# UBC-ECE-Sasha/PIM-compression

Measured on AMD Instinct MI355X. Metric: end-to-end GB/s (compress + decompress) on Silesia-mix; bit-exact ratio parity, higher is better.
Workload: dtype u8; 1 GPU; silesia_mix 8 x 1024 MiB containers in all (BASELINE configs[4]), block_size 32768; containers_this_rank=8, container_bytes=1073741824, block_size=32768, parallelism=whole containers dealt over 1 GPU(s), no collective

## Files before the change

pim-compression_amd/csrc/snappy_k1_stream.hpp:

```cpp
#pragma once

namespace snappy_hip {

#ifdef SNAPPY_EMU
inline unsigned long long g_stream_stats[16] = {0};
#define STREAM_STAT(i) do { if (lane == 0) ++g_stream_stats[i]; } while (0)
#else
#define STREAM_STAT(i) ((void)0)
#endif

#ifdef SNAPPY_PROF
__device__ unsigned long long g_prof[32];
struct StreamProf {
    unsigned long long acc = 0, cnt = 0, last = 0;
};
#define PROF_START() (prof.last = __builtin_readcyclecounter())
#define PROF_LAP(i) do { const unsigned long long now_ = __builtin_readcyclecounter(); if (lane == (i)) { prof.acc += now_ - prof.last; prof.cnt++; } prof.last = now_; } while (0)
#define PROF_WAIT() __builtin_amdgcn_s_waitcnt(0)
#define PROF_FLUSH() do { if (lane < 16) { atomicAdd(&g_prof[lane], prof.acc); atomicAdd(&g_prof[16 + lane], prof.cnt); } } while (0)
#elif defined(SNAPPY_MARK)
struct StreamProf {};
#define PROF_START() asm volatile("; PHASE start")
#define PROF_LAP(i) asm volatile("; PHASE " #i)
#define PROF_WAIT() ((void)0)
#define PROF_FLUSH() ((void)0)
#else
struct StreamProf {};
#define PROF_START() ((void)0)
#define PROF_LAP(i) ((void)0)
#define PROF_WAIT() ((void)0)
#define PROF_FLUSH() ((void)0)
#endif

template <class T, class = void> struct table_gathers_once : std::false_type {};
template <class T> struct table_gathers_once<T, std::void_t<decltype(T::kGathersOnce)>> : std::true_type {};

constexpr uint32_t kStreamRoom = 192;
#ifndef SNAPPY_STREAM_SLOTS_LDS
#define SNAPPY_STREAM_SLOTS_LDS 512
#endif
constexpr uint32_t kStreamSlotsLds = SNAPPY_STREAM_SLOTS_LDS, kStreamSlotsGlobal = 256;
__host__ __device__ constexpr uint32_t stream_scratch_bytes(uint32_t slots) { return 8u * slots; }

struct StreamWindow {
    uint32_t base;
    uint4 a, b;
    uint32_t h0, e0;
};

__device__ __forceinline__ void stream_load_window(StreamWindow& w, const uint8_t* __restrict__ blk, uint32_t base, uint32_t last16,
                                                   uint32_t lane)
{
    w.base = base;
    const uint32_t q = base + lane;
    w.a = ld128(blk + (q < last16 ? q : last16));
    w.b = ld128(blk + (q + 16u < last16 ? q + 16u : last16));
}
__device__ __forceinline__ void stream_hash_window(StreamWindow& w, uint32_t shift)
{
    const uint32_t prod = w.a.x * kHashMul;
    w.h0 = prod >> shift;
    w.e0 = (prod << (32 - shift)) & 0xffff0000u;
}

struct StreamGather {
    uint32_t ent;
    uint4 ka, kb;
    unsigned long long worthm;
};
template <class Table>
__device__ __forceinline__ void stream_issue_gather(StreamGather& g, const Table& table, const StreamWindow& w,
                                                    const uint8_t* __restrict__ blk, uint32_t lane)
{
    const uint32_t mine_l = w.e0 | (w.base + lane);
    g.ent = table.load_lane(w.h0, mine_l);
    const bool worth = !Table::certain_miss(g.ent, mine_l);
    g.worthm = __ballot(worth);
    g.ka = g.kb = make_uint4(0, 0, 0, 0);
    if (worth) {
        const uint8_t* __restrict__ c = blk + (g.ent & 0xffffu);
        g.ka = ld128(c);
        g.kb = ld128(c + 16);
    }
}

#ifdef SNAPPY_EMU
__device__ __forceinline__ uint32_t lds_max_rtn(lds_words_t p, uint32_t v)
{
    const uint32_t old = *p;
    if (v > old) *p = v;
    return old;
}
#else
__device__ __forceinline__ uint32_t lds_max_rtn(lds_words_t p, uint32_t v)
{
    return __hip_atomic_fetch_max((__attribute__((address_space(3))) uint32_t*)p, v, __ATOMIC_RELAXED, __HIP_MEMORY_SCOPE_WAVEFRONT);
}
#endif

struct StreamDup {
    uint32_t j1 = 0;
    uint32_t extj = 0;
    unsigned long long nf = 0;
    unsigned long long hitj = 0;
    unsigned long long deep = 0;
    unsigned long long cx = 0;
};

template <uint32_t kSlots>
__device__ __forceinline__ void stream_analyse(StreamDup& d, const StreamWindow& w, lds_bytes_t scratch, uint32_t lane)
{
    lds_words_t tab = (lds_words_t)scratch;
    const uint32_t sa = w.h0 & (kSlots - 1u);
    const uint32_t sb = kSlots + ((w.h0 >> 5) & (kSlots - 1u));
#ifdef SNAPPY_EMU
    static const bool unordered = getenv("EMU_LDS_UNORDERED") != nullptr;
    uint32_t oa = 0, ob = 0;
    if (unordered) {
        oa = lds_max_rtn(tab + sa, lane + 1u);
        ob = lds_max_rtn(tab + sb, lane + 1u);
    } else {
        for (uint32_t turn = 0; turn < kWave; ++turn) {
            if (lane == turn) {
                oa = lds_max_rtn(tab + sa, lane + 1u);
                ob = lds_max_rtn(tab + sb, lane + 1u);
            }
            __builtin_amdgcn_wave_barrier();
        }
    }
#else
    const uint32_t oa = lds_max_rtn(tab + sa, lane + 1u);
    const uint32_t ob = lds_max_rtn(tab + sb, lane + 1u);
#endif
    __builtin_amdgcn_wave_barrier();
    tab[sa] = 0;
    tab[sb] = 0;
    __builtin_amdgcn_wave_barrier();
    const uint32_t ja = oa - 1u, jb = ob - 1u;
    d = StreamDup();
    if (__ballot((oa && ja >= lane) || (ob && jb >= lane))) {
        STREAM_STAT(7);
        d.cx = dup_slot_lanes(scratch, w.h0, lane);
        for (uint32_t i = lane; i < 2u * kSlots; i += kWave) tab[i] = 0;
        __builtin_amdgcn_wave_barrier();
        return;
    }
    const uint32_t ha = (uint32_t)__shfl((int)w.h0, (int)(ja & 63u));
    const uint32_t hb = (uint32_t)__shfl((int)w.h0, (int)(jb & 63u));
    const unsigned long long OA = __ballot(oa != 0), OB = __ballot(ob != 0);
    const unsigned long long MA = OA & __ballot(ha == w.h0), MB = OB & __ballot(hb == w.h0);
    const bool ma = __builtin_amdgcn_inverse_ballot_w64(MA);
    d.j1 = ma ? ja : jb;
    d.nf = MA | MB;
    d.cx = OA & OB & ~d.nf;
    if (d.nf) {
        const uint32_t jl = d.j1 & 63u;
        const uint32_t xj = (uint32_t)__shfl((int)w.a.x, (int)jl);
        const uint32_t e1 = (uint32_t)__shfl((int)w.a.y, (int)jl) ^ w.a.y;
        const uint32_t e2 = (uint32_t)__shfl((int)w.a.z, (int)jl) ^ w.a.z;
        d.hitj = d.nf & __ballot(xj == w.a.x);
        d.extj = min_u32(min_u32(first_bit(e1), first_bit(e2) | 32u), 64u) >> 3;
        const unsigned long long chained = d.nf | d.cx;
        d.deep = d.nf & __ballot(((uint32_t)(chained >> jl) & 1u) != 0);
    }
}

__device__ __forceinline__ void stream_walk(uint32_t advv, uint32_t clv, uint32_t& t, unsigned long long& V, unsigned long long& COV)
{
#ifdef SNAPPY_EMU
    for (;;) {
        const uint32_t l = t & 63u;
        V |= 1ull << l;
        const uint32_t a = (uint32_t)__builtin_amdgcn_readlane((int)advv, (int)l);
        const uint32_t c = (uint32_t)__builtin_amdgcn_readlane((int)clv, (int)l);
        if (c) COV |= ((1ull << c) - 1ull) << l;
        const uint32_t nt = t + a;
        const bool carry = nt < t;
        t = nt;
        if (carry) break;
    }
#else
    uint32_t a, c;
    unsigned long long m;
    asm volatile(
        "1:\n"
        "  s_bitset1_b64 %[V], %[t]\n"
        "  v_readlane_b32 %[a], %[advv], %[t]\n"
        "  v_readlane_b32 %[c], %[clv], %[t]\n"
        "  s_bfm_b64 %[m], %[c], %[t]\n"
        "  s_or_b64 %[COV], %[COV], %[m]\n"
        "  s_add_u32 %[t], %[t], %[a]\n"
        "  s_cbranch_scc1 2f\n"
        "  s_bitset1_b64 %[V], %[t]\n"
        "  v_readlane_b32 %[a], %[advv], %[t]\n"
        "  v_readlane_b32 %[c], %[clv], %[t]\n"
        "  s_bfm_b64 %[m], %[c], %[t]\n"
        "  s_or_b64 %[COV], %[COV], %[m]\n"
        "  s_add_u32 %[t], %[t], %[a]\n"
        "  s_cbranch_scc1 2f\n"
        "  s_bitset1_b64 %[V], %[t]\n"
        "  v_readlane_b32 %[a], %[advv], %[t]\n"
        "  v_readlane_b32 %[c], %[clv], %[t]\n"
        "  s_bfm_b64 %[m], %[c], %[t]\n"
        "  s_or_b64 %[COV], %[COV], %[m]\n"
        "  s_add_u32 %[t], %[t], %[a]\n"
        "  s_cbranch_scc1 2f\n"
        "  s_bitset1_b64 %[V], %[t]\n"
        "  v_readlane_b32 %[a], %[advv], %[t]\n"
        "  v_readlane_b32 %[c], %[clv], %[t]\n"
        "  s_bfm_b64 %[m], %[c], %[t]\n"
        "  s_or_b64 %[COV], %[COV], %[m]\n"
        "  s_add_u32 %[t], %[t], %[a]\n"
        "  s_cbranch_scc0 1b\n"
        "2:\n"
        : [t] "+s"(t), [V] "+s"(V), [COV] "+s"(COV), [a] "=&s"(a), [c] "=&s"(c), [m] "=&s"(m)
        : [advv] "v"(advv), [clv] "v"(clv)
        : "scc");
#endif
}

#ifndef SNAPPY_EMU
__device__ __forceinline__ unsigned long long uni64(unsigned long long v)
{
    return (unsigned long long)uni((uint32_t)v) | ((unsigned long long)uni((uint32_t)(v >> 32)) << 32);
}
#else
__device__ __forceinline__ unsigned long long uni64(unsigned long long v) { return v; }
#endif

__device__ __forceinline__ uint32_t stream_past(uint32_t dist, unsigned long long inter, uint32_t land)
{
    if (land >= kWave || ((inter >> land) & 1ull)) return 0;
    return (uint32_t)__builtin_amdgcn_readlane((int)dist, (int)land);
}

__device__ __forceinline__ bool has_run_of_34(unsigned long long m)
{
    unsigned long long r = m & (m >> 1);
    r &= r >> 2;
    r &= r >> 4;
    r &= r >> 8;
    r &= r >> 16;
    return (r & (m >> 32) & (m >> 33)) != 0;
}

template <class Table>
__device__ __forceinline__ void stream_put(const Table& table, uint32_t x, uint32_t pos, uint32_t shift, uint32_t lane)
{
    const uint32_t prod = x * kHashMul;
    if constexpr (Table::kCollectiveStore)
        table.store_masked(1ull, prod >> shift, pos, lane);
    else
        table.put(prod >> shift, ((prod << (32 - shift)) & 0xffff0000u) | pos, lane);
}
template <class Table>
__device__ __forceinline__ void stream_store(const Table& table, const StreamWindow& w, unsigned long long m, uint32_t lane)
{
    if constexpr (Table::kCollectiveStore) {
        table.store_masked(m, w.h0, w.base + lane, lane);
    } else {
        if (__builtin_amdgcn_inverse_ballot_w64(m)) table.store_lane(w.h0, w.e0 | (w.base + lane));
        __builtin_amdgcn_wave_barrier();
    }
}

__device__ __forceinline__ void stream_emit(uint8_t* __restrict__ dst, const uint8_t* __restrict__ blk, uint32_t& op, uint32_t& next_emit,
                                            uint32_t base, uint32_t x0, uint32_t ent, uint32_t extv, unsigned long long H,
                                            unsigned long long COV, bool by_copy, uint32_t r_out, bool long_copy, uint32_t ip,
                                            uint32_t long_cand, uint32_t long_len, uint32_t lane)
{
    if (H) emit_segment(dst, blk, op, next_emit, base, x0, ent, extv, H, COV, by_copy, r_out, lane);
    if (long_copy) {
        if (ip > next_emit) op = emit_literal_windowed(dst, op, blk, next_emit, ip - next_emit, base, x0, lane);
        op = emit_copy(dst, op, ip - long_cand, long_len, lane);
        next_emit = ip + long_len;
    }
}

struct SoloMate {
    static constexpr bool kAnalysesInPlace = true;
    __device__ __forceinline__ void begin(uint32_t, uint32_t, uint32_t) {}
    __device__ __forceinline__ void drain(uint32_t&, uint32_t&, uint32_t) {}
    template <uint32_t kSlots>
    __device__ __forceinline__ void analysis(StreamDup& d, const StreamWindow& w, lds_bytes_t scratch, uint32_t lane)
    {
        stream_analyse<kSlots>(d, w, scratch, lane);
    }
    __device__ __forceinline__ void emit(uint8_t* __restrict__ dst, const uint8_t* __restrict__ blk, uint32_t& op, uint32_t& next_emit,
                                         uint32_t base, uint32_t x0, uint32_t ent, uint32_t extv, unsigned long long H,
                                         unsigned long long COV, bool by_copy, uint32_t r_out, bool long_copy, uint32_t ip,
                                         uint32_t long_cand, uint32_t long_len, uint32_t lane)
    {
        stream_emit(dst, blk, op, next_emit, base, x0, ent, extv, H, COV, by_copy, r_out, long_copy, ip, long_cand, long_len, lane);
    }
};

template <class Table, uint32_t kSlots, class Mate>
__device__ __forceinline__ void stream_run(const uint8_t* __restrict__ blk, uint32_t avail, uint32_t n, uint32_t shift,
                                           uint8_t* __restrict__ dst, const Table table, uint32_t lane, lds_bytes_t dup_scratch,
                                           ParseState& ps, StreamProf& prof, Mate& mate)
{
    const uint32_t limit = n - kInputMargin;
    const uint32_t last16 = avail - 16u;
    uint32_t ip = ps.ip, skip = ps.skip, op = ps.op, next_emit = ps.next_emit;
    mate.begin(op, next_emit, lane);

    for (;;) {
        StreamWindow cur, nxt;
        stream_load_window(cur, blk, ip & ~63u, last16, lane);
        stream_hash_window(cur, shift);
        StreamGather g;
        stream_issue_gather(g, table, cur, blk, lane);
        __builtin_amdgcn_sched_barrier(0);
        stream_load_window(nxt, blk, cur.base + 64u, last16, lane);
        StreamDup dup;
        mate.template analysis<kSlots>(dup, cur, dup_scratch, lane);
        PROF_LAP(0);
        bool restart = false;

        for (;;) {
            const uint32_t r0 = ip - cur.base;
            const uint32_t b_in = 64u - skip;
            PROF_WAIT();
            PROF_LAP(1);

            unsigned long long hitm = __ballot(g.ka.x == cur.a.x) & g.worthm;
            const uint32_t t1 = min_u32(first_bit(g.ka.y ^ cur.a.y), first_bit(g.ka.z ^ cur.a.z) | 32u);
            const uint32_t t2 = min_u32(first_bit(g.ka.w ^ cur.a.w), first_bit(g.kb.x ^ cur.b.x) | 32u) | 64u;
            const uint32_t t3 = min_u32(first_bit(g.kb.y ^ cur.b.y), first_bit(g.kb.z ^ cur.b.z) | 32u) | 128u;
            uint32_t extv = min_u32(min_u32(t1, t2), min_u32(t3, 192u)) >> 3;
            uint32_t ent = g.ent & 0xffffu;
            const unsigned long long pend = dup.nf & __ballot(dup.j1 >= r0);
            const unsigned long long satm = hitm & __ballot(extv == 24u);
            unsigned long long stopm = pend | dup.cx | satm;
            const unsigned long long above_r0 = ~0ull << r0;
            const unsigned long long inter = hitm | stopm;
            const unsigned long long up = (lane < 63u) ? (inter >> (lane + 1u)) : 0ull;
            const uint32_t dist = up ? (uint32_t)__builtin_ctzll(up) + 1u : 64u - lane;
            const bool stopl = __builtin_amdgcn_inverse_ballot_w64(stopm);
            const bool hitl = __builtin_amdgcn_inverse_ballot_w64(hitm);
            const uint32_t clt = hitl ? 4u + extv : 0u;
            const bool hitjl = __builtin_amdgcn_inverse_ballot_w64(dup.hitj);
            const uint32_t clj = hitjl ? 4u + dup.extj : 0u;
            const uint32_t land_t = lane + clt, land_j = lane + clj;
            const uint32_t dist_t = (uint32_t)__shfl((int)dist, (int)(land_t & 63u));
            const uint32_t dist_j = (uint32_t)__shfl((int)dist, (int)(land_j & 63u));
            const bool plain_t = land_t < 64u && !((inter >> (land_t & 63u)) & 1ull);
            const bool plain_j = land_j < 64u && !((inter >> (land_j & 63u)) & 1ull);
            const uint32_t advt = hitl ? clt + (plain_t ? dist_t : 0u) : dist;
            const uint32_t advj = hitjl ? clj + (plain_j ? dist_j : 0u) : dist;
            const unsigned long long satjm = dup.hitj & __ballot(dup.extj == 8u);
            uint32_t clv = stopl ? 0u : clt;
            uint32_t advv = stopl ? 64u : advt;
            PROF_LAP(2);

            unsigned long long V = 0, COV = 0;
            uint32_t t = r0 - 64u;
            uint32_t r_out = 0;
            bool long_copy = false;
            uint32_t long_cand = 0, long_len = 0;
            for (;;) {
                t = uni(t);
                stream_walk(advv, clv, t, V, COV);
                const uint32_t s = 63u - (uint32_t)__builtin_clzll(V);
                if (!((stopm >> s) & 1ull)) {
                    r_out = t + 64u;
                    break;
                }
                PROF_LAP(3);
                STREAM_STAT(3);
                const unsigned long long bit_s = 1ull << s;
                const unsigned long long below_s = bit_s - 1ull;
                const unsigned long long interior_s = COV & ~(V & hitm & below_s);
                uint32_t how = 0;
                uint32_t j = 0;
                if (pend & bit_s) {
                    j = (uint32_t)__builtin_amdgcn_readlane((int)dup.j1, (int)s);
                    const unsigned long long not_inserted = interior_s & (interior_s >> 1);
                    if (!((not_inserted >> j) & 1ull)) how = 1;
                    else if (dup.deep & bit_s) how = 2;
                }
                if (dup.cx & bit_s) how = 2;
                uint32_t adv_s, cl_s, cand_s = 0, sat_s = 24;
                bool hit_s, more_s;
                if (how == 2) {
                    STREAM_STAT(6);
                    const unsigned long long ins = ((above_r0 & below_s & ~interior_s) | (COV & ~(interior_s >> 1))) & below_s;
                    const uint32_t hs = (uint32_t)__builtin_amdgcn_readlane((int)cur.h0, (int)s);
                    const unsigned long long J = __ballot(cur.h0 == hs) & ins;
                    how = 0;
                    if (J) {
                        j = 63u - (uint32_t)__builtin_clzll(J);
                        hit_s = (uint32_t)__builtin_amdgcn_readlane((int)cur.a.x, (int)s) == (uint32_t)__builtin_amdgcn_readlane((int)cur.a.x, (int)j);
                        const uint32_t e1 = (uint32_t)__builtin_amdgcn_readlane((int)cur.a.y, (int)s) ^ (uint32_t)__builtin_amdgcn_readlane((int)cur.a.y, (int)j);
                        const uint32_t e2 = (uint32_t)__builtin_amdgcn_readlane((int)cur.a.z, (int)s) ^ (uint32_t)__builtin_amdgcn_readlane((int)cur.a.z, (int)j);
                        const uint32_t ext_s = e1 ? ((uint32_t)__builtin_ctz(e1) >> 3) : (e2 ? 4u + ((uint32_t)__builtin_ctz(e2) >> 3) : 8u);
                        cand_s = cur.base + j;
                        sat_s = 8;
                        more_s = hit_s && ext_s == 8u;
                        cl_s = hit_s ? 4u + ext_s : 0u;
                        adv_s = hit_s ? cl_s : (uint32_t)__builtin_amdgcn_readlane((int)dist, (int)s);
                        if (hit_s && !more_s) adv_s += stream_past(dist, hitm | stopm, s + cl_s);
                        how = 3;
                    }
                }
                if (how == 1) {
                    STREAM_STAT(9);
                    hit_s = (dup.hitj & bit_s) != 0;
                    more_s = (satjm & bit_s) != 0;
                    adv_s = (uint32_t)__builtin_amdgcn_readlane((int)advj, (int)s);
                    cl_s = (uint32_t)__builtin_amdgcn_readlane((int)clj, (int)s);
                    cand_s = cur.base + j;
                    sat_s = 8;
                } else if (how == 0) {
                    STREAM_STAT(10);
                    hit_s = (hitm & bit_s) != 0;
                    more_s = (satm & bit_s) != 0;
                    adv_s = (uint32_t)__builtin_amdgcn_readlane((int)advt, (int)s);
                    cl_s = (uint32_t)__builtin_amdgcn_readlane((int)clt, (int)s);
                }
                if (more_s) {
                    STREAM_STAT(8);
                    if (how == 0) cand_s = (uint32_t)__builtin_amdgcn_readlane((int)ent, (int)s);
                    cl_s = 4u + sat_s + match_extend(blk, cand_s + 4u + sat_s, cur.base + s + 4u + sat_s, n, lane);
                    adv_s = cl_s <= 63u ? cl_s + stream_past(dist, hitm | stopm, s + cl_s) : cl_s;
                    if (cl_s > 63u) {
// ... 156 lines not shown
```

pim-compression_amd/csrc/snappy_kernels.hpp:

```cpp
#pragma once
#include <hip/hip_runtime.h>
#include <type_traits>
#include <stdint.h>
#ifdef SNAPPY_EMU
#include <stdio.h>
#include <stdlib.h>
#endif

#include "snappy_device_common.hpp"

namespace snappy_hip {

constexpr uint32_t kMaxTableEntries = 16384;
constexpr uint32_t kHashMul = 0x1e35a7bdu;
constexpr uint32_t kInputMargin = 15;

#if defined(__HIP_DEVICE_COMPILE__)
#define SNAPPY_PIN(x) asm volatile("" : "+v"(x))
#else
#define SNAPPY_PIN(x) ((void)0)
#endif

constexpr uint32_t kBlockOk = 0;
constexpr uint32_t kBlockInvalid = 1;
constexpr uint32_t kRangeOutOfBounds = 2;

__device__ __forceinline__ uint32_t table_entries_for(uint32_t n)
{
    uint32_t ts = 256;
    while (ts < kMaxTableEntries && ts < n) ts <<= 1;
    return ts;
}


__device__ __forceinline__ uint32_t emit_literal(uint8_t* __restrict__ dst, uint32_t op,
                                                 const uint8_t* __restrict__ src, uint32_t len, uint32_t lane)
{
    const uint32_t n = len - 1;
    uint32_t hdr;
    if (n < 60) {
        hdr = 1;
        if (lane == 0) dst[op] = (uint8_t)(n << 2);
    } else {
        const uint32_t cnt = (n < 256u) ? 1u : ((n < 65536u) ? 2u : 3u);
        hdr = 1 + cnt;
        if (lane < hdr)
            dst[op + lane] = (lane == 0) ? (uint8_t)((59 + cnt) << 2) : (uint8_t)(n >> (8 * (lane - 1)));
    }
    uint8_t* d = dst + op + hdr;
    if (len <= kWave) {
        if (lane < len) d[lane] = src[lane];
    } else {
        uint32_t i = 4 * lane;
        for (; i + 4 <= len; i += 4 * kWave) st32(d + i, ld32(src + i));
        for (; i < len; ++i) d[i] = src[i];
    }
    return op + hdr + len;
}

__device__ __forceinline__ uint32_t emit_copy_piece(uint8_t* __restrict__ dst, uint32_t op, uint32_t off,
                                                    uint32_t len, uint32_t lane)
{
    if (len < 12 && off < 2048) {
        if (lane < 2)
            dst[op + lane] = (lane == 0) ? (uint8_t)(1 + ((len - 4) << 2) + ((off >> 8) << 5)) : (uint8_t)(off & 0xff);
        return op + 2;
    }
    if (lane < 3)
        dst[op + lane] = (lane == 0) ? (uint8_t)(2 + ((len - 1) << 2))
                                     : ((lane == 1) ? (uint8_t)(off & 0xff) : (uint8_t)(off >> 8));
    return op + 3;
}

__device__ __forceinline__ uint32_t emit_copy(uint8_t* __restrict__ dst, uint32_t op, uint32_t off, uint32_t len,
                                              uint32_t lane)
{
    if (len > 64) {
        const uint32_t n64 = (len >= 68) ? ((len - 68) / 64 + 1) : 0;
        len -= 64 * n64;
        const uint32_t has60 = (len > 64) ? 1u : 0u;
        if (has60) len -= 60;
        const uint32_t nfull = n64 + has60;
        for (uint32_t k = lane; k < nfull; k += kWave) {
            const uint32_t plen = (k < n64) ? 64u : 60u;
            uint8_t* p = dst + op + 3 * k;
            p[0] = (uint8_t)(2 + ((plen - 1) << 2));
            p[1] = (uint8_t)(off & 0xff);
            p[2] = (uint8_t)(off >> 8);
        }
        op += 3 * nfull;
    }
    return emit_copy_piece(dst, op, off, len, lane);
}

__device__ __forceinline__ uint32_t match_extend(const uint8_t* __restrict__ blk, uint32_t a, uint32_t b, uint32_t n,
                                                 uint32_t lane)
{
    uint32_t m = 0;
    for (;;) {
        const uint32_t pb = b + m + 4 * lane;
        const uint32_t pa = a + m + 4 * lane;
        uint32_t eq;
        if (pb + 4 <= n) {
            const uint32_t x = ld32(blk + pa) ^ ld32(blk + pb);
            eq = x ? ((uint32_t)__builtin_ctz(x) >> 3) : 4u;
        } else {
            eq = 0;
            for (uint32_t k = 0; pb + k < n; ++k) {
                if (blk[pa + k] != blk[pb + k]) break;
                ++eq;
            }
        }
        const unsigned long long stop = __ballot(eq != 4);
        if (stop == 0) {
            m += 4 * kWave;
            continue;
        }
        const uint32_t first = (uint32_t)__builtin_ctzll(stop);
        return m + 4 * first + (uint32_t)__builtin_amdgcn_readlane((int)eq, (int)first);
    }
}

struct CursorWindow {
    const uint8_t* __restrict__ blk;
    uint32_t avail;
    uint32_t shift;
    uint32_t base;
    uint32_t x0, h0, e0;
    uint32_t x1;

    __device__ __forceinline__ void rehash()
    {
        const uint32_t prod = x0 * kHashMul;
        h0 = prod >> shift;
        e0 = (prod << (32 - shift)) & 0xffff0000u;
    }

    __device__ __forceinline__ uint32_t load_at(uint32_t pos, uint32_t lane) const
    {
        const uint32_t q = pos + lane;
        const uint32_t last = avail - 4;
        return ld32(blk + ((q < last) ? q : last));
    }
    __device__ __forceinline__ void reset(uint32_t pos, uint32_t lane)
    {
        base = pos & ~63u;
        x0 = load_at(base, lane);
        rehash();
        __builtin_amdgcn_sched_barrier(0);
        x1 = load_at(base + 64, lane);
    }
    __device__ __forceinline__ bool ensure(uint32_t pos, uint32_t lane)
    {
        if (pos < base + 64) return false;
        if (pos < base + 128) {
            base += 64;
            x0 = x1;
            rehash();
            __builtin_amdgcn_sched_barrier(0);
            x1 = load_at(base + 64, lane);
        } else {
            reset(pos, lane);
        }
        return true;
    }
    __device__ __forceinline__ uint32_t bytes_at(uint32_t pos) const
    {
        return (uint32_t)__builtin_amdgcn_readlane((int)x0, (int)(pos - base));
    }
    __device__ __forceinline__ uint32_t hash_at(uint32_t pos) const
    {
        return (uint32_t)__builtin_amdgcn_readlane((int)h0, (int)(pos - base));
    }
    __device__ __forceinline__ uint32_t entry_at(uint32_t pos) const
    {
        return (uint32_t)__builtin_amdgcn_readlane((int)e0, (int)(pos - base)) | pos;
    }
    __device__ __forceinline__ uint32_t bytes_near(uint32_t pos) const
    {
        const uint32_t rel = pos - base;
        if (rel < 64) return (uint32_t)__builtin_amdgcn_readlane((int)x0, (int)rel);
        uint32_t v = x1;
        SNAPPY_PIN(v);
        return (uint32_t)__builtin_amdgcn_readlane((int)v, (int)(rel - 64));
    }
};

#ifdef SNAPPY_EMU
typedef volatile uint8_t* lds_bytes_t;
typedef volatile uint32_t* lds_words_t;
__device__ __forceinline__ void lds_or(lds_words_t p, uint32_t v) { *p = *p | v; }
__device__ __forceinline__ void lds_and(lds_words_t p, uint32_t v) { *p = *p & v; }
#else
typedef volatile __attribute__((address_space(3))) uint8_t* lds_bytes_t;
typedef volatile __attribute__((address_space(3))) uint32_t* lds_words_t;
__device__ __forceinline__ void lds_or(lds_words_t p, uint32_t v)
{
    __hip_atomic_fetch_or((__attribute__((address_space(3))) uint32_t*)p, v, __ATOMIC_RELAXED, __HIP_MEMORY_SCOPE_WAVEFRONT);
}
__device__ __forceinline__ void lds_and(lds_words_t p, uint32_t v)
{
    __hip_atomic_fetch_and((__attribute__((address_space(3))) uint32_t*)p, v, __ATOMIC_RELAXED, __HIP_MEMORY_SCOPE_WAVEFRONT);
}
#endif

#ifdef SNAPPY_EMU
__device__ __forceinline__ uint32_t lds_ld32u(lds_bytes_t p)
{
    uint32_t v;
    __builtin_memcpy(&v, (const void*)p, 4);
    return v;
}
__device__ __forceinline__ void lds_st32u(lds_bytes_t p, uint32_t v) { __builtin_memcpy((void*)p, &v, 4); }
#else
typedef uint32_t __attribute__((aligned(1))) lds_u32_unaligned_t;
__device__ __forceinline__ uint32_t lds_ld32u(lds_bytes_t p)
{
    return *reinterpret_cast<volatile __attribute__((address_space(3))) lds_u32_unaligned_t*>(p);
}
__device__ __forceinline__ void lds_st32u(lds_bytes_t p, uint32_t v)
{
    *reinterpret_cast<volatile __attribute__((address_space(3))) lds_u32_unaligned_t*>(p) = v;
}
#endif

#ifdef SNAPPY_EMU
inline uint32_t g_emu_store_index[16][kWave];
__device__ __forceinline__ void emu_check_distinct_stores(bool stores, uint32_t index, uint32_t lane)
{
    uint32_t* mine = g_emu_store_index[blockIdx.x & 15u];
    mine[lane] = stores ? index : 0xffffffffu;
    __builtin_amdgcn_wave_barrier();
    if (stores)
        for (uint32_t l = 0; l < kWave; ++l)
            if (l != lane && mine[l] == index) {
                fprintf(stderr, "emulator: lanes %u and %u store to table entry %u in one instruction\n", lane, l, index);
                abort();
            }
    __builtin_amdgcn_wave_barrier();
}
#else
__device__ __forceinline__ void emu_check_distinct_stores(bool, uint32_t, uint32_t) {}
#endif

struct FilteredGlobalTable {
    static constexpr bool kCollectiveStore = false;
    uint32_t* __restrict__ t;
    lds_words_t written;
    uint32_t empty;
    __device__ __forceinline__ void init(uint32_t entries, uint32_t, uint32_t lane) const
    {
        for (uint32_t i = lane; i < entries / 32; i += kWave) written[i] = 0;
        __builtin_amdgcn_wave_barrier();
    }
    __device__ __forceinline__ bool is_written(uint32_t h) const { return (written[h >> 5] >> (h & 31u)) & 1u; }
    __device__ __forceinline__ uint32_t exchange(uint32_t h, uint32_t entry, uint32_t lane) const
    {
        uint32_t hv = h;
        SNAPPY_PIN(hv);
        uint32_t old = empty;
        if (is_written(hv)) old = t[hv];
        old = uni(old);
        t[hv] = entry;
        if (lane == 0) lds_or(written + (h >> 5), 1u << (h & 31u));
        __builtin_amdgcn_wave_barrier();
        return old;
    }
    __device__ __forceinline__ void put(uint32_t h, uint32_t entry, uint32_t lane) const
    {
        uint32_t hv = h;
        SNAPPY_PIN(hv);
        t[hv] = entry;
        if (lane == 0) lds_or(written + (h >> 5), 1u << (h & 31u));
        __builtin_amdgcn_wave_barrier();
    }
    __device__ __forceinline__ static bool certain_miss(uint32_t old, uint32_t entry) { return ((old ^ entry) >> 16) != 0; }
    __device__ __forceinline__ uint32_t load_lane(uint32_t h, uint32_t = 0) const { return is_written(h) ? t[h] : empty; }
    __device__ __forceinline__ void store_lane(uint32_t h, uint32_t entry) const
    {
        t[h] = entry;
        lds_or(written + (h >> 5), 1u << (h & 31u));
    }
    __device__ __forceinline__ FilteredGlobalTable with_empty(uint32_t e) const { return FilteredGlobalTable{t, written, e}; }
};

template <uint32_t kSlots>
struct CachedGlobalTable {
    static constexpr bool kCollectiveStore = true;
    uint16_t* __restrict__ t;
    lds_words_t written;
    lds_words_t cache;
    __device__ __forceinline__ void init(uint32_t entries, uint32_t, uint32_t lane) const
    {
        for (uint32_t i = lane; i < entries / 32; i += kWave) written[i] = 0;
        for (uint32_t i = lane; i < kSlots; i += kWave) cache[i] = 0;
        __builtin_amdgcn_wave_barrier();
    }
    __device__ __forceinline__ bool is_written(uint32_t h) const { return (written[h >> 5] >> (h & 31u)) & 1u; }
    __device__ __forceinline__ static bool certain_miss(uint32_t, uint32_t) { return false; }
    __device__ __forceinline__ CachedGlobalTable with_empty(uint32_t) const { return *this; }
    __device__ __forceinline__ uint32_t load_lane(uint32_t h, uint32_t mine) const
    {
        const uint32_t w = cache[h & (kSlots - 1u)];
        const bool wr = is_written(h);
        uint32_t pos = w & 0xffffu;
        if ((w >> 16) != h + 1u) pos = wr ? (uint32_t)t[h] : 0u;
        return (mine & 0xffff0000u) | pos;
    }
    __device__ __forceinline__ void store_masked(unsigned long long m, uint32_t h, uint32_t pos, uint32_t lane) const
    {
        const bool s = __builtin_amdgcn_inverse_ballot_w64(m);
        const uint32_t idx = h & (kSlots - 1u), mine = ((h + 1u) << 16) | (pos & 0xffffu);
        const uint32_t old = cache[idx];
        __builtin_amdgcn_wave_barrier();
        if (s) {
            cache[idx] = mine;
            lds_or(written + (h >> 5), 1u << (h & 31u));
        }
        __builtin_amdgcn_wave_barrier();
        const uint32_t now = cache[idx];
        const bool lost = s && now != mine;
        const bool evicts = s && !lost && old != 0u && (old >> 16) != h + 1u;
        if (evicts) t[(old >> 16) - 1u] = (uint16_t)old;
        emu_check_distinct_stores(evicts, (old >> 16) - 1u, lane);
        __builtin_amdgcn_wave_barrier();
        if (__ballot(lost)) {
            if (lost) t[h] = (uint16_t)pos;
            emu_check_distinct_stores(lost, h, lane);
        }
        __builtin_amdgcn_wave_barrier();
    }
};

struct LdsTable {
    static constexpr bool kCollectiveStore = false;
    uint16_t* t;
    __device__ __forceinline__ void init(uint32_t entries, uint32_t, uint32_t lane) const
    {
        uint4* q = reinterpret_cast<uint4*>(t);
        for (uint32_t i = lane; i < entries / 8; i += kWave) q[i] = make_uint4(0, 0, 0, 0);
    }
    __device__ __forceinline__ uint32_t exchange(uint32_t h, uint32_t entry, uint32_t lane) const
    {
        const uint32_t old = uni((uint32_t)t[h]);
        if (lane == 0) t[h] = (uint16_t)entry;
        __builtin_amdgcn_wave_barrier();
        return old;
    }
    __device__ __forceinline__ void put(uint32_t h, uint32_t entry, uint32_t lane) const
    {
        if (lane == 0) t[h] = (uint16_t)entry;
        __builtin_amdgcn_wave_barrier();
    }
    __device__ __forceinline__ static bool certain_miss(uint32_t, uint32_t) { return false; }
    __device__ __forceinline__ uint32_t load_lane(uint32_t h, uint32_t = 0) const { return t[h]; }
    __device__ __forceinline__ void store_lane(uint32_t h, uint32_t entry) const { t[h] = (uint16_t)entry; }
    __device__ __forceinline__ LdsTable with_empty(uint32_t) const { return *this; }
};


__device__ __forceinline__ uint32_t emit_copy_packed(uint8_t* __restrict__ dst, uint32_t op, uint32_t off, uint32_t len,
                                                     uint32_t lane)
{
    if (len > 64) return emit_copy(dst, op, off, len, lane);
    uint32_t word, bytes;
    if (len < 12 && off < 2048) {
        word = (1 + ((len - 4) << 2) + ((off >> 8) << 5)) | ((off & 0xff) << 8);
        bytes = 2;
    } else {
        word = (2 + ((len - 1) << 2)) | (off << 8);
        bytes = 3;
    }
    if (lane == 0) st32(dst + op, word);
    return op + bytes;
}

__device__ __forceinline__ uint32_t emit_literal_windowed(uint8_t* __restrict__ dst, uint32_t op,
                                                          const uint8_t* __restrict__ blk, uint32_t from, uint32_t len,
                                                          uint32_t win_base, uint32_t win_x0, uint32_t lane)
{
    if (from < win_base || from + len > win_base + kWave) return emit_literal(dst, op, blk + from, len, lane);
    const uint32_t n = len - 1;
    uint32_t hdr;
    if (n < 60) {
        hdr = 1;
        if (lane == 0) dst[op] = (uint8_t)(n << 2);
    } else {
        hdr = 2;
        if (lane == 0) {
            dst[op] = (uint8_t)(60 << 2);
            dst[op + 1] = (uint8_t)n;
        }
    }
    const uint32_t rel = from - win_base;
    if (lane >= rel && lane < rel + len) dst[op + hdr + lane - rel] = (uint8_t)win_x0;
    return op + hdr + len;
}

__constant__ uint32_t kRecip16[64] = {
        0, 65537, 32769, 21846, 16385, 13108, 10923,  9363,  8193,  7282,  6554,  5958,  5462,  5042,  4682,  4370,
     4097,  3856,  3641,  3450,  3277,  3121,  2979,  2850,  2731,  2622,  2521,  2428,  2341,  2260,  2185,  2115,
     2049,  1986,  1928,  1873,  1821,  1772,  1725,  1681,  1639,  1599,  1561,  1525,  1490,  1457,  1425,  1395,
     1366,  1338,  1311,  1286,  1261,  1237,  1214,  1192,  1171,  1150,  1130,  1111,  1093,  1075,  1058,  1041};

constexpr uint32_t kDupSlots = 1024;

__device__ __forceinline__ uint32_t first_bit(uint32_t x) { return (uint32_t)__builtin_ffs((int)x) - 1u; }
__device__ __forceinline__ uint32_t min_u32(uint32_t a, uint32_t b) { return a < b ? a : b; }

__device__ __forceinline__ uint32_t ctz64_or(unsigned long long x, uint32_t if_zero)
{
    return x ? (uint32_t)__builtin_ctzll(x) : if_zero;
}
__device__ __forceinline__ unsigned long long lane_range(uint32_t lo, uint32_t cnt)
{
    return (~0ull >> (64u - cnt)) << lo;
}

__device__ __forceinline__ unsigned long long dup_slot_lanes(lds_bytes_t scratch, uint32_t h, uint32_t lane)
{
    const uint32_t sa = h & (kDupSlots / 2 - 1);
    const uint32_t sb = kDupSlots / 2 + ((h >> 5) & (kDupSlots / 2 - 1));
    scratch[sa] = (uint8_t)lane;
    scratch[sb] = (uint8_t)lane;
    __builtin_amdgcn_wave_barrier();
    const uint32_t wa = scratch[sa];
    const uint32_t wb = scratch[sb];
    __builtin_amdgcn_wave_barrier();
    if (wa != lane) scratch[sa] = 0xff;
    if (wb != lane) scratch[sb] = 0xff;
    __builtin_amdgcn_wave_barrier();
    const uint32_t ma = scratch[sa];
    const uint32_t mb = scratch[sb];
    __builtin_amdgcn_wave_barrier();
    return __ballot(ma == 0xff && mb == 0xff);
}

template <class Table, uint32_t kChunk>
struct MaskedWindowState {
    uint32_t ent = 0;
    uint32_t extv = 0;
    unsigned long long hit = 0;
    unsigned long long dup = 0;
    unsigned long long longm = 0;
    unsigned long long deepm = 0;
    unsigned long long inserted = 0;
    uint32_t xa = 0, xb = 0;
    uint32_t cov_end = 0;
    bool dup_valid = false;

    __device__ __forceinline__ void invalidate()
    {
        cov_end = 0;
        hit = 0;
        dup_valid = false;
        inserted = 0;
    }

    __device__ __forceinline__ static uint32_t bytes_ahead(const CursorWindow& win, uint32_t lane, uint32_t d)
    {
        const uint32_t src = (lane + d) & 63u;
        const uint32_t a = (uint32_t)__shfl((int)win.x0, (int)src);
        const uint32_t b = (uint32_t)__shfl((int)win.x1, (int)src);
        return (lane + d < kWave) ? a : b;
    }

    template <bool kWithDup = false, bool kDeep = false>
    __device__ __forceinline__ void gather(const Table& table, const CursorWindow& win, lds_bytes_t scratch, uint32_t r,
                                           uint32_t span, uint32_t lane, uint32_t block_len = 0)
    {
        const uint32_t e = (r + span < kWave) ? r + span : kWave;
        if (!kWithDup && !dup_valid) {
            dup = dup_slot_lanes(scratch, win.h0, lane);
            dup_valid = true;
        }
        const unsigned long long gm = kWithDup ? lane_range(r, e - r) : (lane_range(r, e - r) & ~dup);
        const bool g = __builtin_amdgcn_inverse_ballot_w64(gm);
        const uint32_t mine_l = win.e0 | (win.base + lane);
        if (g) ent = table.load_lane(win.h0, mine_l);
        constexpr bool kDupUnderCandidates = std::is_same<Table, LdsTable>::value;
        if (kWithDup && !dup_valid && !kDupUnderCandidates) {
            __builtin_amdgcn_sched_barrier(0);
            dup = dup_slot_lanes(scratch, win.h0, lane);
            dup_valid = true;
            __builtin_amdgcn_sched_barrier(0);
        }
        const bool worth = g && !Table::certain_miss(ent, mine_l);
        uint32_t k0 = 0, k1 = 0, k2 = 0;
        const bool deep = kDeep && worth && (win.base + lane + 28u <= block_len);
        uint32_t k3 = 0, k4 = 0, k5 = 0, k6 = 0, o3 = 1, o4 = 1, o5 = 1, o6 = 1;
        if (worth) {
            const uint8_t* __restrict__ c = win.blk + (ent & 0xffffu);
            k0 = ld32(c);
            k1 = ld32(c + 4);
            k2 = ld32(c + 8);
            if (deep) {
                k3 = ld32(c + 12);
                k4 = ld32(c + 16);
                k5 = ld32(c + 20);
                k6 = ld32(c + 24);
                const uint8_t* __restrict__ o = win.blk + win.base + lane;
                o3 = ld32(o + 12);
                o4 = ld32(o + 16);
                o5 = ld32(o + 20);
                o6 = ld32(o + 24);
            }
        }
        if (kWithDup && !dup_valid && kDupUnderCandidates) {
            __builtin_amdgcn_sched_barrier(0);
            dup = dup_slot_lanes(scratch, win.h0, lane);
            dup_valid = true;
            __builtin_amdgcn_sched_barrier(0);
        }
        xa = bytes_ahead(win, lane, 4);
        xb = bytes_ahead(win, lane, 8);
        const uint32_t t1 = min_u32(first_bit(k1 ^ xa), first_bit(k2 ^ xb) | 32u);
        uint32_t bits = min_u32(t1, 64u);
        if (kDeep) {
            const uint32_t t2 = min_u32(first_bit(k3 ^ o3), first_bit(k4 ^ o4) | 32u) | 64u;
            const uint32_t t3 = min_u32(first_bit(k5 ^ o5), first_bit(k6 ^ o6) | 32u) | 128u;
            bits = min_u32(min_u32(t1, t2), min_u32(t3, 192u));
        }
        extv = bits >> 3;
        const unsigned long long worthm = __ballot(worth);
        deepm = kDeep ? (worthm & __ballot(win.base + lane + 28u <= block_len)) : 0ull;
        hit = worthm & __ballot(k0 == win.x0);
        longm = hit & ((deepm & __ballot(extv == 24u)) | (~deepm & __ballot(extv == 8u)));
        cov_end = e;
    }

    __device__ __forceinline__ static void commit(const Table& table, const CursorWindow& win, unsigned long long m, uint32_t lane)
    {
        if constexpr (Table::kCollectiveStore) {
            table.store_masked(m, win.h0, win.base + lane, lane);
        } else {
            if (__builtin_amdgcn_inverse_ballot_w64(m)) table.store_lane(win.h0, win.e0 | (win.base + lane));
            __builtin_amdgcn_wave_barrier();
        }
    }
};

__device__ __forceinline__ uint32_t mbcnt64(unsigned long long m, uint32_t add)
{
    return (uint32_t)__builtin_amdgcn_mbcnt_hi((uint32_t)(m >> 32), __builtin_amdgcn_mbcnt_lo((uint32_t)m, add));
}
__device__ __forceinline__ unsigned long long lanes_below(uint32_t n) { return ~0ull >> (64u - n); }

__device__ __forceinline__ void emit_segment(uint8_t* __restrict__ dst, const uint8_t* __restrict__ blk, uint32_t& op, uint32_t& next_emit,
                                             uint32_t base, uint32_t x0, uint32_t ent, uint32_t extv, unsigned long long H,
                                             unsigned long long COV, bool by_copy, uint32_t r, uint32_t lane)
{
    const uint32_t r_end = r < kWave ? r : kWave;
    const uint32_t first_hit = (uint32_t)__builtin_ctzll(H);
    const uint32_t last_end = by_copy ? r_end : 64u - (uint32_t)__builtin_clzll(COV);
    uint32_t s0 = first_hit;
    const uint32_t p0 = base + first_hit;
    if (next_emit >= base && p0 - next_emit <= 60u) {
        s0 = next_emit - base;
    } else if (p0 > next_emit) {
        op = emit_literal_windowed(dst, op, blk, next_emit, p0 - next_emit, base, x0, lane);
    }
    const unsigned long long LIT = ((~0ull << s0) & lanes_below(last_end)) & ~COV;
    const unsigned long long LS = LIT & ~(LIT << 1);
    const uint32_t off = base + lane - (ent & 0xffffu);
    const uint32_t len = 4u + extv;
    const bool is_hit = __builtin_amdgcn_inverse_ballot_w64(H);
    const bool three = off >= 2048u || len >= 12u;
    const unsigned long long H3 = __ballot(is_hit && three);
    uint32_t P = mbcnt64(H, 0);
    P = mbcnt64(LIT, op + 2u * P);
    P = mbcnt64(H3, P);
    P = mbcnt64(LS, P);
    const bool is_ls = __builtin_amdgcn_inverse_ballot_w64(LS);
    if (__builtin_amdgcn_inverse_ballot_w64(LIT)) dst[P + (is_ls ? 1u : 0u)] = (uint8_t)x0;
    if (is_ls) {
        const uint32_t runlen = (uint32_t)__builtin_ctzll(~LIT >> lane);
        dst[P] = (uint8_t)((runlen - 1) << 2);
    }
    if (is_hit) {
        uint32_t b0;
        if (!three) b0 = 1u + ((len - 4u) << 2) + ((off >> 8) << 5);
        else b0 = 2u + ((len - 1u) << 2);
        dst[P] = (uint8_t)b0;
        dst[P + 1] = (uint8_t)off;
        if (three) dst[P + 2] = (uint8_t)(off >> 8);
    }
    op += (uint32_t)__builtin_popcountll(LIT) + 2u * (uint32_t)__builtin_popcountll(H) + (uint32_t)__builtin_popcountll(H3) +
          (uint32_t)__builtin_popcountll(LS);
    next_emit = base + (by_copy ? r : last_end);
}

__device__ __forceinline__ uint32_t segment_walk(unsigned long long inter, unsigned long long stopm, uint32_t lenv, uint32_t hi,
                                                 uint32_t& r, uint32_t& B, unsigned long long& H, unsigned long long& COV)
{
    uint32_t why;
#ifdef SNAPPY_EMU
    for (;;) {
        const unsigned long long m = inter >> r;
        const uint32_t f = m ? (uint32_t)__builtin_ctzll(m) : 0xffffffffu;
        if (f >= B) {
            why = 1;
            break;
        }
        r += f;
        B -= f;
        if ((stopm >> r) & 1ull) {
            why = 2;
            break;
        }
        H |= 1ull << r;
        const uint32_t e = (uint32_t)__builtin_amdgcn_readlane((int)lenv, (int)r);
        COV |= ((1ull << e) - 1ull) << r;
        r += e;
        B = 33;
        if (r < hi) continue;
        why = 0;
        break;
    }
#else
    unsigned long long m;
    uint32_t f, e;
    asm volatile(
        "1:\n"
        "  s_lshr_b64 %[m], %[inter], %[r]\n"
        "  s_ff1_i32_b64 %[f], %[m]\n"
        "  s_cmp_ge_u32 %[f], %[B]\n"
        "  s_cbranch_scc1 2f\n"
        "  s_add_u32 %[r], %[r], %[f]\n"
        "  s_sub_u32 %[B], %[B], %[f]\n"
        "  s_bitcmp1_b64 %[stopm], %[r]\n"
        "  s_cbranch_scc1 3f\n"
        "  s_bitset1_b64 %[H], %[r]\n"
        "  v_readlane_b32 %[e], %[lenv], %[r]\n"
        "  s_bfm_b64 %[m], %[e], %[r]\n"
        "  s_or_b64 %[COV], %[COV], %[m]\n"
        "  s_add_u32 %[r], %[r], %[e]\n"
        "  s_movk_i32 %[B], 33\n"
        "  s_cmp_lt_u32 %[r], %[hi]\n"
        "  s_cbranch_scc1 1b\n"
        "  s_mov_b32 %[why], 0\n"
        "  s_branch 4f\n"
        "2:\n"
        "  s_mov_b32 %[why], 1\n"
        "  s_branch 4f\n"
        "3:\n"
        "  s_mov_b32 %[why], 2\n"
        "4:\n"
        : [r] "+s"(r), [B] "+s"(B), [H] "+s"(H), [COV] "+s"(COV), [m] "=&s"(m), [f] "=&s"(f), [e] "=&s"(e), [why] "=&s"(why)
        : [inter] "s"(inter), [stopm] "s"(stopm), [lenv] "v"(lenv), [hi] "s"(hi)
        : "scc");
#endif
    return why;
}

struct ParseState {
    uint32_t ip = 1;
    uint32_t skip = 32;
    uint32_t op = 4;
    uint32_t next_emit = 0;
};

template <class Table, uint32_t kChunk, bool kAtWindowEntry = false>
__device__ __forceinline__ bool bulk_run(const uint8_t* __restrict__ blk, uint32_t avail, uint32_t n, uint32_t shift,
                                         uint8_t* __restrict__ dst, const Table table, uint32_t lane, lds_bytes_t dup_scratch,
                                         ParseState& ps, uint32_t stop_ip)
{
    using State = MaskedWindowState<Table, kChunk>;
    uint32_t op = ps.op;
    uint32_t next_emit = ps.next_emit;
    bool finished = true;
    {
        const uint32_t limit = n - kInputMargin;
        CursorWindow win;
        win.blk = blk;
        win.avail = avail;
        win.shift = shift;
        win.reset(ps.ip, lane);
        State st;
        uint32_t ip = ps.ip;
        uint32_t skip = ps.skip;
        for (uint32_t iter = 0;; ++iter) {
            const uint32_t stride = skip >> 5;
            const uint32_t step = stride ? stride : 1u;
            if (ip + step > limit) break;
            if (iter && ip >= stop_ip && skip < 64u && (!kAtWindowEntry || ip >= win.base + 64u)) {
                finished = false;
                break;
            }
            if (win.ensure(ip, lane)) st.invalidate();
            uint32_t r = ip - win.base;
            if (r >= uni(st.cov_end)) st.template gather<true, true>(table, win, dup_scratch, r, kChunk, lane, n);
            unsigned long long stopm = st.dup | st.longm;

            bool need_single = true;
            if (stride <= 1 || !((stopm >> r) & 1ull)) {
                uint32_t hi = uni(st.cov_end);
                const uint32_t lim = limit - win.base;
                hi = lim < hi ? lim : hi;
                if (hi < kWave) stopm |= ~0ull << hi;
                unsigned long long inter = st.hit | stopm;
                unsigned long long pre = 0;
                uint32_t B = 64u - skip;
                if (stride > 1) {
                    const uint32_t x = lane - r;
                    bool mine = lane == r;
                    if (stride < kWave) {
                        const uint32_t q = (x * kRecip16[stride]) >> 16;
                        mine = lane >= r && x == q * stride;
                    }
                    const uint32_t nrem = 32u - (skip & 31u);
                    uint32_t hs = r + nrem * stride;
                    hs = hs < hi ? hs : hi;
                    const uint32_t lims = lim - (stride - 1u);
                    hs = hs < lims ? hs : lims;
                    const unsigned long long smask = __ballot(mine) & lanes_below(hs);
                    const unsigned long long m = inter & smask;
                    const uint32_t p = ctz64_or(m, kWave);
                    pre = p < kWave ? (p ? smask & lanes_below(p) : 0ull) : smask;
                    const uint32_t cnt = (uint32_t)__builtin_popcountll(pre);
                    skip += cnt;
                    if (p == kWave || ((stopm >> p) & 1ull)) {
                        State::commit(table, win, pre, lane);
                        st.inserted |= pre;
                        ip += cnt * stride;
                        continue;
                    }
                    r = p;
                    B = 1;
                }
                const uint32_t r0 = r;
                unsigned long long H = 0, COV = 0;
                uint32_t why;
                need_single = false;
                for (;;) {
                    why = segment_walk(inter, stopm, 4u + st.extv, hi, r, B, H, COV);
                    if (why != 2 || r >= hi) break;
                    bool hit_r;
                    uint32_t cand_r, ext_r;
                    uint32_t sat_r = 8;
                    if ((st.dup >> r) & 1ull) {
                        const uint32_t hr = (uint32_t)__builtin_amdgcn_readlane((int)win.h0, (int)r);
                        const unsigned long long inner = COV & ~H;
                        const unsigned long long so_far = st.inserted | pre | (((~0ull << r0) & ((1ull << r) - 1ull)) & ~inner) |
                                                          (COV & ~(inner >> 1));
                        const unsigned long long J = __ballot(win.h0 == hr) & so_far & ((1ull << r) - 1ull);
                        if (J) {
                            const uint32_t j = 63u - (uint32_t)__builtin_clzll(J);
                            cand_r = win.base + j;
                            hit_r = (uint32_t)__builtin_amdgcn_readlane((int)win.x0, (int)r) ==
                                    (uint32_t)__builtin_amdgcn_readlane((int)win.x0, (int)j);
                            const uint32_t d0 = (uint32_t)__builtin_amdgcn_readlane((int)st.xa, (int)r) ^
                                                (uint32_t)__builtin_amdgcn_readlane((int)st.xa, (int)j);
                            const uint32_t d1 = (uint32_t)__builtin_amdgcn_readlane((int)st.xb, (int)r) ^
                                                (uint32_t)__builtin_amdgcn_readlane((int)st.xb, (int)j);
                            ext_r = d0 ? ((uint32_t)__builtin_ctz(d0) >> 3) : (d1 ? 4u + ((uint32_t)__builtin_ctz(d1) >> 3) : 8u);
                        } else {
                            hit_r = (st.hit >> r) & 1ull;
                            cand_r = (uint32_t)__builtin_amdgcn_readlane((int)st.ent, (int)r) & 0xffffu;
                            ext_r = (uint32_t)__builtin_amdgcn_readlane((int)st.extv, (int)r);
                            sat_r = ((st.deepm >> r) & 1ull) ? 24u : 8u;
                        }
                    } else {
                        hit_r = true;
                        cand_r = (uint32_t)__builtin_amdgcn_readlane((int)st.ent, (int)r) & 0xffffu;
                        sat_r = ((st.deepm >> r) & 1ull) ? 24u : 8u;
                        ext_r = sat_r;
                    }
                    uint32_t len_r = 4u + ext_r;
                    if (hit_r && ext_r == sat_r)
                        len_r = 4u + sat_r + match_extend(blk, cand_r + 4u + sat_r, win.base + r + 4u + sat_r, n, lane);
                    if (hit_r && len_r > 63u) {
                        need_single = true;
                        break;
                    }
                    if (lane == r) {
                        st.extv = len_r - 4u;
                        st.ent = cand_r;
                    }
                    stopm &= ~(1ull << r);
                    inter = hit_r ? (inter | (1ull << r)) : (inter & ~(1ull << r));
                }
                if (why == 1) {
                    const uint32_t room = hi - r;
                    const uint32_t adv = B < room ? B : room;
                    r += adv;
                    B -= adv;
                }
                ip = win.base + r;
                skip = 64u - B;
                const bool done = (why == 0) && ip >= limit;
                const uint32_t r_end = r < kWave ? r : kWave;

                const unsigned long long interior = COV & ~H;
                const unsigned long long walked = r_end > r0 ? ((~0ull << r0) & lanes_below(r_end)) : 0ull;
                unsigned long long C = pre | (walked & ~interior);
                unsigned long long endl = COV & ~(interior >> 1);
                if (why == 0 && (r > kWave || done)) endl &= ~(1ull << (r_end - 1));
                C |= endl;
                State::commit(table, win, C & ~st.dup, lane);
                st.inserted |= C;
                for (unsigned long long d = C & st.dup; d; d &= d - 1)
                    State::commit(table, win, d & (~d + 1), lane);

                if (H) emit_segment(dst, blk, op, next_emit, win.base, win.x0, st.ent, st.extv, H, COV, why == 0, r, lane);
                if (done) break;
                if (why == 0 && r > kWave) {
                    if (win.ensure(ip - 1, lane)) st.invalidate();
                    State::commit(table, win, 1ull << (ip - 1 - win.base), lane);
                    st.inserted |= 1ull << (ip - 1 - win.base);
                }
                if (!need_single) continue;
                r = ip - win.base;
            }

            uint32_t cand = 0, ext = 0, sat = 8;
            bool hit;
            unsigned long long J = 0;
            if ((st.dup >> r) & 1ull) {
                const uint32_t hr = win.hash_at(ip);
                J = __ballot(win.h0 == hr) & st.inserted & ((1ull << r) - 1ull);
            }
            State::commit(table, win, 1ull << r, lane);
            st.inserted |= 1ull << r;
            if (J) {
                const uint32_t j = 63u - (uint32_t)__builtin_clzll(J);
                cand = win.base + j;
                hit = win.bytes_at(ip) == (uint32_t)__builtin_amdgcn_readlane((int)win.x0, (int)j);
                if (hit) {
                    const uint32_t d0 = (uint32_t)__builtin_amdgcn_readlane((int)st.xa, (int)r) ^
                                        (uint32_t)__builtin_amdgcn_readlane((int)st.xa, (int)j);
                    const uint32_t d1 = (uint32_t)__builtin_amdgcn_readlane((int)st.xb, (int)r) ^
                                        (uint32_t)__builtin_amdgcn_readlane((int)st.xb, (int)j);
                    ext = d0 ? ((uint32_t)__builtin_ctz(d0) >> 3) : (d1 ? 4u + ((uint32_t)__builtin_ctz(d1) >> 3) : 8u);
                }
            } else {
                hit = (st.hit >> r) & 1ull;
                if (hit) {
                    cand = (uint32_t)__builtin_amdgcn_readlane((int)st.ent, (int)r) & 0xffffu;
                    ext = (uint32_t)__builtin_amdgcn_readlane((int)st.extv, (int)r);
                    sat = ((st.deepm >> r) & 1ull) ? 24u : 8u;
                }
// ... 976 lines not shown
```

Baseline: 63.14 GB/s.

## Batch strided skip-scan across wave lanes and widen long literal copies

Adds a strided_scan_batch path that, when the skip stride is at least 2, evaluates up to 64 future probe positions in parallel (one per lane), handling hash lookups, duplicate-slot detection and table stores collectively. It then advances ip past all misses at once instead of stepping one probe per loop iteration. Separately, long literals (>=1024 bytes) are copied with unrolled 128-bit loads and stores; the streaming emitter opts out via a template flag. This targets the serial cost of incompressible regions, at the cost of extra LDS barriers and possible wasted work when a hit occurs early in the batch.

```diff
diff --git a/pim-compression_amd/csrc/snappy_k1_stream.hpp b/pim-compression_amd/csrc/snappy_k1_stream.hpp
--- a/pim-compression_amd/csrc/snappy_k1_stream.hpp
+++ b/pim-compression_amd/csrc/snappy_k1_stream.hpp
@@ -2,12 +2,6 @@
 
 namespace snappy_hip {
 
-#ifdef SNAPPY_EMU
-inline unsigned long long g_stream_stats[16] = {0};
-#define STREAM_STAT(i) do { if (lane == 0) ++g_stream_stats[i]; } while (0)
-#else
-#define STREAM_STAT(i) ((void)0)
-#endif
 
 #ifdef SNAPPY_PROF
 __device__ unsigned long long g_prof[32];
@@ -269,9 +263,9 @@
                                             unsigned long long COV, bool by_copy, uint32_t r_out, bool long_copy, uint32_t ip,
                                             uint32_t long_cand, uint32_t long_len, uint32_t lane)
 {
-    if (H) emit_segment(dst, blk, op, next_emit, base, x0, ent, extv, H, COV, by_copy, r_out, lane);
+    if (H) emit_segment<false>(dst, blk, op, next_emit, base, x0, ent, extv, H, COV, by_copy, r_out, lane);
     if (long_copy) {
-        if (ip > next_emit) op = emit_literal_windowed(dst, op, blk, next_emit, ip - next_emit, base, x0, lane);
+        if (ip > next_emit) op = emit_literal_windowed<false>(dst, op, blk, next_emit, ip - next_emit, base, x0, lane);
         op = emit_copy(dst, op, ip - long_cand, long_len, lane);
         next_emit = ip + long_len;
     }
diff --git a/pim-compression_amd/csrc/snappy_kernels.hpp b/pim-compression_amd/csrc/snappy_kernels.hpp
--- a/pim-compression_amd/csrc/snappy_kernels.hpp
+++ b/pim-compression_amd/csrc/snappy_kernels.hpp
@@ -33,6 +33,7 @@
 }
 
 
+template <bool kWide = true>
 __device__ __forceinline__ uint32_t emit_literal(uint8_t* __restrict__ dst, uint32_t op,
                                                  const uint8_t* __restrict__ src, uint32_t len, uint32_t lane)
 {
@@ -50,6 +51,23 @@
     uint8_t* d = dst + op + hdr;
     if (len <= kWave) {
         if (lane < len) d[lane] = src[lane];
+    } else if (kWide && len >= 1024u) {
+        uint32_t base = 0;
+        for (; base + 64u * kWave <= len; base += 64u * kWave) {
+            const uint8_t* __restrict__ s = src + (base + 16u * lane);
+            uint8_t* __restrict__ t = d + (base + 16u * lane);
+            const uint4 v0 = ld128(s), v1 = ld128(s + 16u * kWave), v2 = ld128(s + 32u * kWave), v3 = ld128(s + 48u * kWave);
+            st128(t, v0);
+            st128(t + 16u * kWave, v1);
+            st128(t + 32u * kWave, v2);
+            st128(t + 48u * kWave, v3);
+        }
+        const uint32_t last = len - 16u;
+        for (; base < len; base += 16u * kWave) {
+            const uint32_t i = base + 16u * lane;
+            const uint32_t o = i < last ? i : last;
+            st128(d + o, ld128(src + o));
+        }
     } else {
         uint32_t i = 4 * lane;
         for (; i + 4 <= len; i += 4 * kWave) st32(d + i, ld32(src + i));
@@ -243,6 +261,13 @@
 __device__ __forceinline__ void emu_check_distinct_stores(bool, uint32_t, uint32_t) {}
 #endif
 
+#ifdef SNAPPY_EMU
+inline unsigned long long g_stream_stats[16] = {0};
+#define STREAM_STAT(i) do { if (lane == 0) ++g_stream_stats[i]; } while (0)
+#else
+#define STREAM_STAT(i) ((void)0)
+#endif
+
 struct FilteredGlobalTable {
     static constexpr bool kCollectiveStore = false;
     uint32_t* __restrict__ t;
@@ -375,11 +400,12 @@
     return op + bytes;
 }
 
+template <bool kWide = true>
 __device__ __forceinline__ uint32_t emit_literal_windowed(uint8_t* __restrict__ dst, uint32_t op,
                                                           const uint8_t* __restrict__ blk, uint32_t from, uint32_t len,
                                                           uint32_t win_base, uint32_t win_x0, uint32_t lane)
 {
-    if (from < win_base || from + len > win_base + kWave) return emit_literal(dst, op, blk + from, len, lane);
+    if (from < win_base || from + len > win_base + kWave) return emit_literal<kWide>(dst, op, blk + from, len, lane);
     const uint32_t n = len - 1;
     uint32_t hdr;
     if (n < 60) {
@@ -434,6 +460,100 @@
     const uint32_t mb = scratch[sb];
     __builtin_amdgcn_wave_barrier();
     return __ballot(ma == 0xff && mb == 0xff);
+}
+__device__ __forceinline__ unsigned long long dup_slot_lanes_among(lds_bytes_t scratch, uint32_t h, bool on, uint32_t lane)
+{
+    const uint32_t sa = h & (kDupSlots / 2 - 1);
+    const uint32_t sb = kDupSlots / 2 + ((h >> 5) & (kDupSlots / 2 - 1));
+    if (on) {
+        scratch[sa] = (uint8_t)lane;
+        scratch[sb] = (uint8_t)lane;
+    }
+    __builtin_amdgcn_wave_barrier();
+    uint32_t wa = lane, wb = lane;
+    if (on) {
+        wa = scratch[sa];
+        wb = scratch[sb];
+    }
+    __builtin_amdgcn_wave_barrier();
+    if (wa != lane) scratch[sa] = 0xff;
+    if (wb != lane) scratch[sb] = 0xff;
+    __builtin_amdgcn_wave_barrier();
+    uint32_t ma = 0, mb = 0;
+    if (on) {
+        ma = scratch[sa];
+        mb = scratch[sb];
+    }
+    __builtin_amdgcn_wave_barrier();
+    return __ballot(ma == 0xff && mb == 0xff);
+}
+
+template <class Table>
+__device__ __forceinline__ uint32_t strided_scan_batch(const Table& table, const uint8_t* __restrict__ blk, uint32_t shift,
+                                                       uint32_t limit, uint32_t ip, uint32_t skip, lds_bytes_t dup_scratch,
+                                                       uint32_t lane, uint32_t& ip_out, bool& again)
+{
+    const uint32_t stride0 = skip >> 5;
+    const uint32_t c0 = 32u - (skip & 31u);
+    const uint32_t over0 = lane > c0 ? lane - c0 : 0u;
+    const uint32_t over1 = lane > c0 + 32u ? lane - c0 - 32u : 0u;
+    const uint32_t pk = ip + lane * stride0 + over0 + over1;
+    const uint32_t stride_k = (skip + lane) >> 5;
+    const bool live = pk + stride_k <= limit;
+    const unsigned long long livem = __ballot(live);
+    const uint32_t x = ld32(blk + (live ? pk : ip));
+    const uint32_t prod = x * kHashMul;
+    const uint32_t h = prod >> shift;
+    const uint32_t mine = ((prod << (32 - shift)) & 0xffff0000u) | pk;
+    uint32_t ent = 0;
+    if (live) ent = table.load_lane(h, mine);
+    const unsigned long long dupm = dup_slot_lanes_among(dup_scratch, h, live, lane);
+    const bool worth = live && !Table::certain_miss(ent, mine);
+    uint32_t k0 = 0;
+    if (worth) k0 = ld32(blk + (ent & 0xffffu));
+    const unsigned long long hitm = __ballot(worth) & __ballot(k0 == x);
+    unsigned long long stops = hitm | dupm | ~livem;
+    uint32_t m;
+    again = true;
+    STREAM_STAT(11);
+    for (;;) {
+        m = ctz64_or(stops, kWave);
+        if (m == kWave) {
+            STREAM_STAT(15);
+            break;
+        }
+        if (!((livem >> m) & 1ull)) {
+            STREAM_STAT(14);
+            break;
+        }
+        if ((dupm >> m) & 1ull) {
+            const uint32_t hm = (uint32_t)__builtin_amdgcn_readlane((int)h, (int)m);
+            if (m && (__ballot(h == hm) & livem & lane_range(0, m))) {
+                STREAM_STAT(13);
+                break;
+            }
+        }
+        if ((hitm >> m) & 1ull) {
+            STREAM_STAT(12);
+            again = false;
+            break;
+        }
+        stops &= ~(1ull << m);
+    }
+    ip_out = m < kWave ? (uint32_t)__builtin_amdgcn_readlane((int)pk, (int)m)
+                       : (uint32_t)__builtin_amdgcn_readlane((int)pk, 63) + ((skip + 63u) >> 5);
+    if (m) {
+        const unsigned long long cm = lane_range(0, m);
+        if constexpr (Table::kCollectiveStore) {
+            table.store_masked(cm, h, pk, lane);
+        } else {
+            const bool s = __builtin_amdgcn_inverse_ballot_w64(cm);
+            if (s) table.store_lane(h, mine);
+            emu_check_distinct_stores(s, h, lane);
+            __builtin_amdgcn_wave_barrier();
+        }
+    }
+    return m;
 }
 
 template <class Table, uint32_t kChunk>
@@ -546,6 +666,7 @@
 }
 __device__ __forceinline__ unsigned long long lanes_below(uint32_t n) { return ~0ull >> (64u - n); }
 
+template <bool kWide = true>
 __device__ __forceinline__ void emit_segment(uint8_t* __restrict__ dst, const uint8_t* __restrict__ blk, uint32_t& op, uint32_t& next_emit,
                                              uint32_t base, uint32_t x0, uint32_t ent, uint32_t extv, unsigned long long H,
                                              unsigned long long COV, bool by_copy, uint32_t r, uint32_t lane)
@@ -558,7 +679,7 @@
     if (next_emit >= base && p0 - next_emit <= 60u) {
         s0 = next_emit - base;
     } else if (p0 > next_emit) {
-        op = emit_literal_windowed(dst, op, blk, next_emit, p0 - next_emit, base, x0, lane);
+        op = emit_literal_windowed<kWide>(dst, op, blk, next_emit, p0 - next_emit, base, x0, lane);
     }
     const unsigned long long LIT = ((~0ull << s0) & lanes_below(last_end)) & ~COV;
     const unsigned long long LS = LIT & ~(LIT << 1);
@@ -679,6 +800,7 @@
         State st;
         uint32_t ip = ps.ip;
         uint32_t skip = ps.skip;
+        bool batch_ok = true;
         for (uint32_t iter = 0;; ++iter) {
             const uint32_t stride = skip >> 5;
             const uint32_t step = stride ? stride : 1u;
@@ -687,6 +809,17 @@
                 finished = false;
                 break;
             }
+            if (!kAtWindowEntry && stride >= 2u && batch_ok) {
+                uint32_t ip_m;
+                const uint32_t m = strided_scan_batch(table, blk, shift, limit, ip, skip, dup_scratch, lane, ip_m, batch_ok);
+                if (m) {
+                    ip = ip_m;
+                    skip += m;
+                    st.invalidate();
+                    continue;
+                }
+            }
+            batch_ok = true;
             if (win.ensure(ip, lane)) st.invalidate();
             uint32_t r = ip - win.base;
             if (r >= uni(st.cov_end)) st.template gather<true, true>(table, win, dup_scratch, r, kChunk, lane, n);
```

New measurement: 65.10 GB/s (median of 6 runs). 3.1% higher.
